# microsoft/DirectXTex

Measured on AMD Instinct MI355X. Metric: Mtexels/s BC7 encode (4096^2 RGBA8, TEX_COMPRESS_DEFAULT), higher is better.
Workload: dtype fp32 seed fit + i32 exact error sums (u8 texels in, 128-bit blocks out); 1 GPU; cfg2: 4096x4096 RGBA8 -> BC7_UNORM, TEX_COMPRESS_DEFAULT, one image per GPU, source and payload resident in HBM (dxtex_compress_device)

## Files before the change

directxtex_amd/csrc/bc7_encode.hip:

```cpp
#include "dxtex_kernels.h"
#include "bc67_tables.h"
#include "bc7_core.h"
#include "search_common.h"
#include <algorithm>
#include <cstdio>
#include <cstdlib>
#include <vector>

namespace dxtex
{
namespace
{
using namespace bc7;

struct Cand { uint32_t err; uint32_t ord; uint64_t lo, hi; };

enum : int { SLOT_M0 = 0, SLOT_M1, SLOT_M2, SLOT_M3, SLOT_M4A, SLOT_M4B, SLOT_M5, SLOT_M6, SLOT_M7, NUM_SLOTS };
enum : int { LIST_BYTES = 64 };

enum : int { PHASE_ALL = 0, PHASE_EARLY = 1, PHASE_LATE = 2 };

struct Bc7Args
{
    SegTable seg;
    uint32_t nblocks;
    uint32_t flags;
    uint8_t* lists;
    Cand* cands;
    uint32_t* px;
    struct TaskRec* recs;
    uint2* order;
    uint32_t* tinfo;
    uint32_t* counters;
    uint32_t* zeroOrd;
    uint2* seeds1;
    uint2* seeds3;
    uint2* seeds;
    int* bestErr;
    int prune;
    int alias;
    uint32_t* aliased;
    const uint32_t* flagged;
    uint32_t early6Min;
    uint32_t earlyAlphaMin;
    int early6Pct;
    int phase;
    const uint32_t* gate;
    uint32_t gateMin;
    uint32_t perturbWaveMax;
    uint32_t exhWaveMax;
};

constexpr uint32_t kWaveTaskMax = 262144;
constexpr uint32_t kWaveTaskMax45 = 24576;
constexpr uint32_t kPerturbWaveMax = 32768;

__device__ __forceinline__ void load_block_texel(const SrcView& src, uint32_t nbw, uint32_t nb, uint32_t t, float* f4, uint32_t& ldr)
{
    const uint32_t by = nb / nbw, bx = nb - by * nbw;
    const uint32_t x0 = bx * 4, y0 = by * 4;
    const uint32_t pw = min(4u, src.width - x0), ph = min(4u, src.height - y0);
    const uint32_t sx = x0 + replicate_src(t & 3, pw), sy = y0 + replicate_src(t >> 2, ph);
    const Texel px = convert_texel(load_texel(src.pixels + uint64_t(sy) * src.rowPitch, sx, src.format), src.tcv, src.tsw);
    f4[0] = px.r; f4[1] = px.g; f4[2] = px.b; f4[3] = px.a;
    const float c[4] = { px.r, px.g, px.b, px.a };
    ldr = 0;
#pragma unroll
    for (int i = 0; i < 4; ++i)
    {
        float v = c[i] * 255.0f + 0.01f;
        v = (v < 255.0f) ? v : 255.0f;
        v = (0.0f < v) ? v : 0.0f;
        ldr |= (uint32_t(v) & 0xFFu) << (8 * i);
    }
}

#if !defined(DXTEX_ROUGH_WGS)
#define DXTEX_ROUGH_WGS 8
#endif
__global__ void __launch_bounds__(256, DXTEX_ROUGH_WGS) bc7_rough_kernel(Bc7Args a)
{
    __shared__ float sF[4][64];
    __shared__ uint32_t sL[4][16];
    __shared__ uint2 sSeed[4][128];
    __shared__ int2 sErr[4][128];
    __shared__ uint32_t sOpaque[4];
    const int wave = threadIdx.x >> 6, lane = threadIdx.x & 63;
    const uint32_t nb = blockIdx.x * 4 + wave;
    const bool inRange = nb < a.nblocks;

    if (inRange && lane < 16)
    {
        uint32_t ldr;
        const BcSeg& sg = seg_of(a.seg, nb);
        load_block_texel(sg.src, sg.nbw, sg.nb0 + (nb - sg.l0), lane, &sF[wave][lane * 4], ldr);
        sL[wave][lane] = ldr;
        a.px[uint64_t(nb) * 16 + lane] = ldr;
        if (lane == 0) { a.zeroOrd[nb] = 0xFFFFFFFFu; a.bestErr[nb] = 0x7FFFFFFF; }
    }
    {
        const bool one = !inRange || lane >= 16 || sF[wave][(lane & 15) * 4 + 3] == 1.0f;
        const unsigned long long all = __ballot(one);
        if (lane == 0) sOpaque[wave] = (all == ~0ull) ? 1u : 0u;
    }
    __syncthreads();

    {
        const uint32_t blk = uint32_t(lane) >> 4, ent = uint32_t(lane) & 15u;
        const uint32_t nbk = blockIdx.x * 4 + blk;
        const float* fpxk = sF[blk];
        const uint32_t* pixk = sL[blk];
        const bool opaque = sOpaque[blk] != 0u;
#pragma unroll 1
        for (int k = 0; k < 2; ++k)
        {
            const uint32_t group = k ? uint32_t(7 - wave) : uint32_t(wave);
            const uint32_t code = kFit2Order[group * 16 + ent];
            if (nbk < a.nblocks)
            {
                const uint32_t m1 = kPart2Mask[code >> 1];
                const uint32_t m = (code & 1u) ? m1 : ((~m1) & 0xFFFFu);
                Region rg; region_init(rg, pixk, m);
                uint32_t A, B;
                if (rg.np == 1) { A = pixk[rg.pos(0)]; B = A; }
                else if (rg.np == 2) { A = pixk[rg.pos(0)]; B = pixk[rg.pos(1)]; }
                else if (opaque) seed_endpoints<true, false, true>(fpxk, m, A, B);
                else seed_endpoints<true>(fpxk, m, A, B);
                sSeed[blk][code] = make_uint2(A, B);
#if defined(DXTEX_ROUGH_SPLIT_ERR)
                sErr[blk][code] = make_int2(rough_error<3, 0>(rg, A, B), rough_error<2, 0>(rg, A, B));
#else
                int e3, e2;
                rough_error_3_2(rg, A, B, e3, e2);
                sErr[blk][code] = make_int2(e3, e2);
#endif
            }
        }
    }
    __syncthreads();
    if (!inRange) return;
    const float* fpx = sF[wave];
    const uint32_t* pix = sL[wave];

    const bool alphaLane = (lane < 16) && ((pix[lane & 15] >> 24) != 0xFFu);
    const bool hasAlpha = __ballot(alphaLane) != 0ull;

    uint8_t* lst = a.lists + uint64_t(nb) * LIST_BYTES;

    {
        const uint32_t shape = lane;
        const int2 er0 = sErr[wave][shape * 2], er1 = sErr[wave][shape * 2 + 1];
        const int e3 = er0.x + er1.x, e2 = er0.y + er1.y;
        int ea = e3, eb = e2;
        uint32_t sa = shape, sb = shape;
        for (int i = 0; i < 16; ++i)
        {
            selection_pass(ea, sa, lane, i);
            selection_pass(eb, sb, lane, i);
        }
        if (lane < 16) { lst[lane] = uint8_t(sa); lst[16 + lane] = uint8_t(sb); }
        {
            wave_lds_sync();
            uint32_t ranked2 = uint32_t(__shfl(int(sb), lane & 15));
            asm volatile("" : "+v"(ranked2));
            const uint32_t mine = (lane < 16) ? sa : ranked2;
            if (lane < 32)
            {
                const uint2 s0 = sSeed[wave][mine * 2], s1 = sSeed[wave][mine * 2 + 1];
                reinterpret_cast<uint4*>(a.seeds + uint64_t(nb) * 64)[lane] = make_uint4(s0.x, s0.y, s1.x, s1.y);
            }
        }
        if (lane == 0)
        {
            lst[32] = hasAlpha ? 1 : 0;
            *reinterpret_cast<int*>(lst + 56) = ea;
        }
    }

    if (a.flags & BCF_USE_3SUBSETS)
    {
        const uint32_t shape = lane;
        const uint32_t bits = kPart3Bits[shape];
        int e3 = 0, e2 = 0;
#pragma unroll 1
        for (uint32_t r = 0; r < 3; ++r)
        {
            uint32_t m = 0;
            for (int i = 0; i < 16; ++i) if (((bits >> (2 * i)) & 3u) == r) m |= 1u << i;
            Region rg; region_init(rg, pix, m);
            uint32_t A, B;
            if (rg.np == 1) { A = pix[rg.pos(0)]; B = A; }
            else if (rg.np == 2) { A = pix[rg.pos(0)]; B = pix[rg.pos(1)]; }
            else seed_endpoints<true>(fpx, m, A, B);
            a.seeds3[uint64_t(nb) * 192 + shape * 3 + r] = make_uint2(A, B);
            e3 += rough_error<3, 0>(rg, A, B);
            e2 += rough_error<2, 0>(rg, A, B);
        }
        int ea = (lane < 16) ? e3 : 0x7FFFFFFF, eb = e2;
        uint32_t sa = shape, sb = shape;
        for (int i = 0; i < 16; ++i)
        {
            if (i < 4) selection_pass(ea, sa, lane, i);
            selection_pass(eb, sb, lane, i);
        }
        if (lane < 4) lst[33 + lane] = uint8_t(sa);
        if (lane < 16) lst[40 + lane] = uint8_t(sb);
    }
}

struct TaskRec { uint32_t A, B; int err; int orgErr; };

template<int MODE, int IM> struct TaskMap
{
    typedef ModeInfo<MODE> MI;
    enum : int { NS = MI::NS,
                 G = (NS == 1) ? 1 : (NS == 2) ? 2 : 4,
                 RANKS = (NS == 1) ? ((MODE == 6) ? 1 : 4) : ((MODE == 0) ? 4 : 16),
                 TPB = RANKS * G,
                 LIST = (MODE == 1) ? 0 : (MODE == 0) ? 33 : (MODE == 2) ? 40 : 16,
                 SLOT = (MODE == 0) ? SLOT_M0 : (MODE == 1) ? SLOT_M1 : (MODE == 2) ? SLOT_M2 : (MODE == 3) ? SLOT_M3 :
                        (MODE == 4) ? (IM ? SLOT_M4B : SLOT_M4A) : (MODE == 5) ? SLOT_M5 : (MODE == 6) ? SLOT_M6 : SLOT_M7 };
};

template<int MODE, int IM>
__device__ __forceinline__ uint32_t candidate_sub(uint32_t rank)
{
    return (TaskMap<MODE, IM>::NS == 1) ? ((MODE == 4) ? (rank * 2 + IM) * 16u : rank * 16u) : rank;
}
template<int MODE, int IM>
__device__ __forceinline__ uint32_t candidate_ord(uint32_t rank) { return uint32_t(MODE) * 128u + candidate_sub<MODE, IM>(rank); }

template<int MODE>
__device__ __forceinline__ bool phase_owns(const Bc7Args& a, uint32_t nb)
{
    if (a.phase == PHASE_ALL || (MODE != 4 && MODE != 5 && MODE != 6)) return true;
    const uint8_t* lst = a.lists + uint64_t(nb) * LIST_BYTES;
    const bool early = (MODE == 6) ? (lst[37] != 0 && a.flagged[0] >= a.early6Min) : (lst[32] != 0 && a.flagged[1] >= a.earlyAlphaMin);
    return early == (a.phase == PHASE_EARLY);
}

__device__ __forceinline__ bool lst_has_alpha(const Bc7Args& a, uint32_t nb) { return a.lists[uint64_t(nb) * LIST_BYTES + 32] != 0; }

template<int MODE, int IM>
__device__ __forceinline__ bool task_geometry(const Bc7Args& a, uint32_t nb, uint32_t r, uint32_t& shape, uint32_t& mask, uint32_t& anchor, uint32_t& rot)
{
    typedef TaskMap<MODE, IM> TM;
    shape = 0; mask = 0xFFFFu; anchor = 0; rot = 0;
    if (nb >= a.nblocks) return false;
    if (!phase_owns<MODE>(a, nb)) return false;
    const uint32_t rank = r / TM::G, region = r % TM::G;
    if (a.zeroOrd[nb] < candidate_ord<MODE, IM>(rank)) return false;
    if (TM::NS == 1) { rot = (MODE == 6) ? 0u : r; return true; }
    if (region >= uint32_t(TM::NS)) return false;
    const uint8_t* lst = a.lists + uint64_t(nb) * LIST_BYTES;
    if (MODE == 7 && lst[32] == 0) return false;
    shape = lst[TM::LIST + rank];
    if (TM::NS == 2)
    {
        const uint32_t m1 = kPart2Mask[shape];
        mask = region ? m1 : ((~m1) & 0xFFFFu);
        anchor = region ? uint32_t(kAnchor2[shape]) : 0u;
    }
    else
    {
        const uint32_t bits = kPart3Bits[shape];
        mask = 0;
#pragma unroll
        for (int i = 0; i < 16; ++i) if (((bits >> (2 * i)) & 3u) == region) mask |= 1u << i;
        anchor = (region == 0) ? 0u : (region == 1) ? uint32_t(kAnchor3[shape] & 15) : uint32_t(kAnchor3[shape] >> 4);
    }
    return true;
}

template<int MODE, int IM, bool ASSIGN = true>
__device__ __forceinline__ void task_org(const float* fpx, const uint32_t* pix, uint32_t mask, uint32_t anchor, uint32_t rot,
                                         SubsetResult& res, int& np, bool wantRegion, Region& rgOut, Block16& b16Out, const uint2* seed = nullptr)
{
    typedef TaskMap<MODE, IM> TM;
    if (TM::NS == 1)
    {
        block16_init(b16Out, pix, rot);
        uint32_t A, B;
        if (seed) { const uint2 sd = seed[(MODE == 6) ? 1 : 0]; A = sd.x; B = sd.y; }
        else if (MODE == 6) seed_endpoints<true>(fpx, 0xFFFFu, A, B);
        else seed_endpoints<false>(fpx, 0xFFFFu, A, B);
        if (MODE != 6)
        {
            uint32_t mn = 255, mx = 0;
#pragma unroll
            for (int i = 0; i < 16; ++i) { const uint32_t al = b16Out.px[i] >> 24; mn = min(mn, al); mx = max(mx, al); }
            A = (A & 0x00FFFFFFu) | (mn << 24);
            B = (B & 0x00FFFFFFu) | (mx << 24);
        }
        if (ASSIGN) refine_pre_err<MODE, IM>(b16Out, A, B, 0u, res);
        else fix_pbits<MODE>(quantize_endpoint<MODE>(A), quantize_endpoint<MODE>(B), res.orgA, res.orgB);
        np = 16;
    }
    else
    {
        region_init(rgOut, pix, mask);
        uint32_t A, B;
        if (seed) { const uint2 sd = *seed; A = sd.x; B = sd.y; }
        else if (rgOut.np == 1) { A = pix[rgOut.pos(0)]; B = A; }
        else if (rgOut.np == 2) { A = pix[rgOut.pos(0)]; B = pix[rgOut.pos(1)]; }
        else seed_endpoints<true>(fpx, mask, A, B);
        if (ASSIGN) refine_pre_err<MODE, IM>(rgOut, A, B, anchor, res);
        else fix_pbits<MODE>(quantize_endpoint<MODE>(A), quantize_endpoint<MODE>(B), res.orgA, res.orgB);
        np = rgOut.np;
    }
}

template<int BPW>
__device__ __forceinline__ void stage_packed(const Bc7Args& a, uint32_t nbFirst, int lane, uint32_t* sL)
{
    for (int t = lane; t < BPW * 16; t += 64)
    {
        const uint32_t nb = nbFirst + (uint32_t(t) >> 4);
        sL[t] = (nb < a.nblocks) ? a.px[uint64_t(nb) * 16 + (t & 15)] : 0u;
    }
    wave_lds_sync();
}

#if !defined(DXTEX_PP45_WGS)
#define DXTEX_PP45_WGS 1
#endif
template<int MODE, int IM>
__global__ void __launch_bounds__(256, (MODE == 4 || MODE == 5) ? DXTEX_PP45_WGS : 1) bc7_pre_kernel(Bc7Args a)
{
    typedef TaskMap<MODE, IM> TM;
    constexpr int BPW = (TM::TPB >= 64) ? 1 : 64 / TM::TPB;
    __shared__ uint32_t sL[4][BPW * 16];
// ... 758 lines not shown
__global__ void __launch_bounds__(64) bc7_exhaustive_wave_kernel(Bc7Args a)
{
    typedef LoopCfg<MODE, IM, CHSET> C;
    typedef TaskMap<MODE, IM> TM;
    static_assert(TM::NS == 1, "whole-block tasks only");
    __shared__ uint32_t sTex[16 * kSlotStride];
    const int lane = threadIdx.x;
    const uint32_t live = a.counters[34];
    if (live == 0 || live > a.exhWaveMax) return;
    for (uint32_t idx = blockIdx.x; idx < live; idx += gridDim.x)
    {
        const uint2 task = a.order[idx];
        const TaskRec rec = a.recs[task.x];
        SlotRegion rg;
        wave_lds_sync();
        search_pickup<MODE, IM>(a, task, &sTex[0], rg);
        wave_lds_sync();
        int other;
        const int base = loop_base<MODE, IM, CHSET>(rg, rec.A, rec.B, &other);
        if (loop_is_settled<CHSET>(rec.err, other)) continue;
        ExhState st; st.optA = rec.A; st.optB = rec.B; st.optErr = rec.err;
        st.o = st.i = st.oEnd = st.iEnd = st.lo = 0; st.iA = 0; st.o0 = 0; st.aleb = 0; st.omin = st.imin = 0; st.best = rec.err; st.bestCode = -1; st.ch = C::CH0;
        VarPal<C::N> vp;
#pragma unroll 1
        for (int ch = C::CH0; ch < C::CH1; ++ch)
        {
            st = exh_window<MODE, IM, CHSET>(st, ch);
            if (st.ch >= C::CH1) break;
            varpal_init<MODE, IM, CHSET>(vp, st.optA, st.optB, ch);
            const int oStart = st.o;
            uint64_t bestKey = ~0ull;
#pragma unroll 1
            for (int round = 0; round < 2; ++round)
            {
                const int c = lane + 64 * round;
                const int o = oStart + c / 11, i = st.lo + c % 11;
                const bool valid = c < 121 && o < st.oEnd && i < st.iEnd && i >= o;
                int e = 0x7FFFFFFF;
                if (valid)
                {
                    const int av = st.aleb ? o : i, bv = st.aleb ? i : o;
                    e = eval_var<MODE, IM, CHSET>(rg, vp, ch, unq1<C::PREC>(uint32_t(av)), unq1<C::PREC>(uint32_t(bv)), base);
                }
                const uint64_t key = valid ? ((uint64_t(uint32_t(e)) << 8) | uint32_t(c)) : ~0ull;
                bestKey = key < bestKey ? key : bestKey;
            }
#pragma unroll
            for (int d = 32; d > 0; d >>= 1)
            {
                const uint32_t lo = uint32_t(__shfl_xor(int(uint32_t(bestKey)), d)), hi = uint32_t(__shfl_xor(int(uint32_t(bestKey >> 32)), d));
                const uint64_t other = (uint64_t(hi) << 32) | lo;
                bestKey = other < bestKey ? other : bestKey;
            }
            if (bestKey != ~0ull)
            {
                const int e = int(uint32_t(bestKey >> 8)), c = int(bestKey & 0xFFu);
                if (e < st.best) { st.best = e; st.omin = oStart + c / 11; st.imin = st.lo + c % 11; }
            }
            st = exh_commit(st);
        }
        if (lane == 0)
        {
            TaskRec* r = a.recs + task.x;
            r->A = st.optA; r->B = st.optB; r->err = st.optErr;
        }
    }
}

template<int MODE, int IM>
__global__ void __launch_bounds__(256, (MODE == 4 || MODE == 5) ? DXTEX_PP45_WGS : 1) bc7_post_kernel(Bc7Args a)
{
    typedef TaskMap<MODE, IM> TM;
    constexpr int BPW = (TM::TPB >= 64) ? 1 : 64 / TM::TPB;
    __shared__ uint32_t sL[4][BPW * 16];
    const int wave = threadIdx.x >> 6, lane = threadIdx.x & 63;
    const uint32_t nbFirst = (blockIdx.x * 4 + wave) * BPW;
    if (nbFirst >= a.nblocks) return;
    if (a.gate && *a.gate < a.gateMin) return;
    const uint32_t blk = uint32_t(lane) / TM::TPB, r = uint32_t(lane) % TM::TPB;
    const uint32_t nb = nbFirst + blk;
    const uint32_t rank = r / TM::G, region = r % TM::G;
    uint32_t shape, mask, anchor, rot;
    const bool active = (blk < uint32_t(BPW)) && task_geometry<MODE, IM>(a, nb, r, shape, mask, anchor, rot);
    const bool mine = blk < uint32_t(BPW) && nb < a.nblocks && phase_owns<MODE>(a, nb);
    if (!__any(active))
    {
        if (mine && r == 0)
        {
            Cand c; c.err = 0xFFFFFFFFu; c.ord = 0xFFFFFFFFu; c.lo = 0; c.hi = 0;
            a.cands[uint64_t(nb) * NUM_SLOTS + TM::SLOT] = c;
        }
        return;
    }
    stage_packed<BPW>(a, nbFirst, lane, sL[wave]);

    SubsetResult res;
    res.orgErr = 0; res.optErr = 0; res.orgA = res.orgB = res.optA = res.optB = 0;
    res.orgIdx1 = res.orgIdx2 = res.optIdx1 = res.optIdx2 = 0;
    int np = 0; Region rg; Block16 b16;
    if (active)
    {
        task_org<MODE, IM, false>(nullptr, &sL[wave][blk * 16], mask, anchor, rot, res, np, true, rg, b16,
                                  (TM::NS == 2) ? a.seeds + uint64_t(nb) * 64 + (TM::LIST ? 32 : 0) + r
                                                : (TM::NS == 1) ? a.seeds1 + uint64_t(nb) * 2 : a.seeds3 + uint64_t(nb) * 192 + shape * 3 + (r % TM::G));
        TaskRec rec = a.recs[uint64_t(nb) * TM::TPB + r];
        if constexpr (TM::NS >= 2)
        {
            const uint32_t leader = (a.tinfo[uint64_t(nb) * TM::TPB + r] >> 18) & 63u;
            if (leader)
            {
                const TaskRec lead = a.recs[uint64_t(nb) * TM::TPB + (leader - 1u)];
                rec.A = lead.A; rec.B = lead.B;
            }
        }
        res.orgErr = rec.orgErr;
        if (TM::NS == 1) refine_post<MODE, IM>(b16, rec.A, rec.B, 0u, res);
        else refine_post<MODE, IM>(rg, rec.A, rec.B, anchor, res);
    }
    int orgTot = res.orgErr, optTot = res.optErr;
#pragma unroll
    for (int d = 1; d < TM::G; d <<= 1) { orgTot += __shfl_xor(orgTot, d); optTot += __shfl_xor(optTot, d); }
    const bool useOpt = optTot < orgTot;
    const int err = useOpt ? optTot : orgTot;
    const uint32_t sub = candidate_sub<MODE, IM>(rank);
    const uint32_t key = active ? ((uint32_t(err) << 7) | sub) : 0xFFFFFFFFu;
    uint32_t best = key;
#pragma unroll
    for (int d = 1; d < TM::TPB && d < 64; d <<= 1) best = min(best, uint32_t(__shfl_xor(int(best), d)));
    const bool needOrg = active && key == best && !useOpt;
    if (__any(needOrg))
    {
        if (needOrg)
        {
            if (TM::NS == 1) (void)assign_indices<MODE, IM>(b16, res.orgA, res.orgB, 0u, res.orgIdx1, res.orgIdx2);
            else (void)assign_indices<MODE, IM>(rg, res.orgA, res.orgB, anchor, res.orgIdx1, res.orgIdx2);
        }
    }
    const uint32_t myA = useOpt ? res.optA : res.orgA, myB = useOpt ? res.optB : res.orgB;
    const uint64_t myIdx1 = useOpt ? res.optIdx1 : res.orgIdx1, myIdx2 = useOpt ? res.optIdx2 : res.orgIdx2;
    uint32_t epA[3] = { myA, 0, 0 }, epB[3] = { myB, 0, 0 };
    uint64_t idx1 = myIdx1;
#pragma unroll
    for (int s = 1; s < TM::NS; ++s)
    {
        epA[s] = uint32_t(__shfl_down(int(myA), s));
        epB[s] = uint32_t(__shfl_down(int(myB), s));
        const uint64_t oi = uint64_t(uint32_t(__shfl_down(int(uint32_t(myIdx1)), s))) |
                            (uint64_t(uint32_t(__shfl_down(int(uint32_t(myIdx1 >> 32)), s))) << 32);
        idx1 |= oi;
    }

    if (blk < uint32_t(BPW) && nb < a.nblocks && region == 0)
    {
        if (active && key == best)
        {
            uint32_t anchors[3] = { 0, 0, 0 };
            if (TM::NS == 2) anchors[1] = kAnchor2[shape];
            if (TM::NS == 3) { anchors[1] = kAnchor3[shape] & 15; anchors[2] = kAnchor3[shape] >> 4; }
            Cand c;
            c.err = uint32_t(err);
            c.ord = uint32_t(MODE) * 128u + sub;
            emit_block<MODE>(shape, rot, IM, epA, epB, idx1, myIdx2, anchors, c.lo, c.hi);
            a.cands[uint64_t(nb) * NUM_SLOTS + TM::SLOT] = c;
            if (err == 0) atomicMin(&a.zeroOrd[nb], c.ord);
            atomicMin(&a.bestErr[nb], err);
        }
        else if (!active && rank == 0 && mine)
        {
            Cand c; c.err = 0xFFFFFFFFu; c.ord = 0xFFFFFFFFu; c.lo = 0; c.hi = 0;
            a.cands[uint64_t(nb) * NUM_SLOTS + TM::SLOT] = c;
        }
    }
}

template<bool RGBA>
__global__ void __launch_bounds__(256) bc7_block_seeds_kernel(Bc7Args a)
{
    const uint32_t nb = blockIdx.x * 256u + threadIdx.x;
    if (nb >= a.nblocks) return;
    const BcSeg& sg = seg_of(a.seg, nb);
    float f[64];
#pragma unroll
    for (int t = 0; t < 16; ++t) { uint32_t ldr; load_block_texel(sg.src, sg.nbw, sg.nb0 + (nb - sg.l0), uint32_t(t), &f[t * 4], ldr); }
    uint32_t A, B;
    seed_endpoints<RGBA, true>(f, 0xFFFFu, A, B);
    a.seeds1[uint64_t(nb) * 2 + (RGBA ? 1 : 0)] = make_uint2(A, B);
}

__global__ void __launch_bounds__(256) bc7_flag_count_kernel(Bc7Args a, uint32_t* out)
{
    uint32_t n = 0, m = 0;
    for (uint32_t nb = blockIdx.x * 256u + threadIdx.x; nb < a.nblocks; nb += gridDim.x * 256u)
    {
        uint8_t* lst = a.lists + uint64_t(nb) * LIST_BYTES;
        const bool hasAlpha = lst[32] != 0;
        bool first = hasAlpha;
        if (!first)
        {
            const uint4* px4 = reinterpret_cast<const uint4*>(a.px + uint64_t(nb) * 16);
            const uint4 q0 = px4[0], q1 = px4[1], q2 = px4[2], q3 = px4[3];
            const uint32_t px[16] = { q0.x, q0.y, q0.z, q0.w, q1.x, q1.y, q1.z, q1.w, q2.x, q2.y, q2.z, q2.w, q3.x, q3.y, q3.z, q3.w };
            const int ea = *reinterpret_cast<const int*>(lst + 56);
            first = int64_t(subset_lower_bound(px, 0xFFFFu, 0u, 4)) * 100 <= int64_t(ea) * a.early6Pct;
        }
        lst[37] = first ? 1 : 0;
        n += first ? 1u : 0u;
        m += hasAlpha ? 1u : 0u;
    }
#pragma unroll
    for (int o = 32; o > 0; o >>= 1) { n += __shfl_xor(n, o); m += __shfl_xor(m, o); }
    if ((threadIdx.x & 63u) == 0 && n) atomicAdd(out, n);
    if ((threadIdx.x & 63u) == 0 && m) atomicAdd(out + 1, m);
}

__global__ void __launch_bounds__(256) bc7_texels_kernel(Bc7Args a)
{
    const uint32_t i = blockIdx.x * 256u + threadIdx.x;
    if (i >= a.nblocks * 16u) return;
    float f4[4]; uint32_t ldr;
    const BcSeg& sg = seg_of(a.seg, i >> 4);
    load_block_texel(sg.src, sg.nbw, sg.nb0 + ((i >> 4) - sg.l0), i & 15u, f4, ldr);
    a.px[i] = ldr;
    if ((i & 15u) == 0) { a.zeroOrd[i >> 4] = 0xFFFFFFFFu; a.bestErr[i >> 4] = 0x7FFFFFFF; }
}

__global__ void __launch_bounds__(256) bc7_pick_kernel(Bc7Args a, uint32_t slotMask)
{
    const uint32_t nb = blockIdx.x * 256u + threadIdx.x;
    if (nb >= a.nblocks) return;
    const Cand* c = a.cands + uint64_t(nb) * NUM_SLOTS;
    uint64_t bestKey = ~0ull;
    uint64_t lo = 0, hi = 0;
#pragma unroll
    for (int s = 0; s < NUM_SLOTS; ++s)
    {
        if (!((slotMask >> s) & 1u)) continue;
        if (s == SLOT_M7 && a.flagged[1] == 0) continue;
        const Cand v = c[s];
        if (v.err == 0xFFFFFFFFu) continue;
        const uint64_t key = (uint64_t(v.err) << 32) | v.ord;
        if (key < bestKey) { bestKey = key; lo = v.lo; hi = v.hi; }
    }
    const BcSeg& sg = seg_of(a.seg, nb);
    const uint32_t gb = sg.nb0 + (nb - sg.l0);
    const uint32_t by = gb / sg.nbw, bx = gb - by * sg.nbw;
    uint64_t* out = reinterpret_cast<uint64_t*>(sg.dst + uint64_t(by) * sg.dstRowPitch) + 2 * uint64_t(bx);
    out[0] = lo; out[1] = hi;
}
}

namespace
{
const uint64_t kMaxBlocksPerPass = dev_env("DXTEX_MAX_BLOCKS_PER_PASS") ? std::max<uint64_t>(1, strtoull(dev_env("DXTEX_MAX_BLOCKS_PER_PASS"), nullptr, 10)) : (1u << 22);
constexpr int kMaxTasksPerBlock = 64;
const uint64_t kSmallPassBlocks = dev_env("DXTEX_BC7_SMALL_BLOCKS") ? strtoull(dev_env("DXTEX_BC7_SMALL_BLOCKS"), nullptr, 10) : 262144;
struct ScratchLayout
{
    size_t lists, cands, px, recs, order, tinfo, counters, zeroOrd, bestErr, seeds, seeds1, seeds3, flagcnt, auxRecs, auxOrder, auxTinfo, auxCounters, total;
    size_t auxTpb, auxSlices;
    explicit ScratchLayout(uint64_t nb, bool threeSubsets)
    {
        auto up = [](size_t v) { return (v + 255) & ~size_t(255); };
        const size_t tpb = threeSubsets ? kMaxTasksPerBlock : 32;
        const bool small = nb <= kSmallPassBlocks;
        auxTpb = small ? tpb : 4; auxSlices = small ? size_t(kSideStreams) : 2;
        size_t o = 0;
        lists = o; o = up(o + nb * LIST_BYTES);
        cands = o; o = up(o + nb * NUM_SLOTS * sizeof(Cand));
        px = o; o = up(o + nb * 64);
        recs = o; o = up(o + nb * tpb * sizeof(TaskRec));
        order = o; o = up(o + nb * tpb * sizeof(uint2));
        tinfo = o; o = up(o + nb * tpb * sizeof(uint32_t));
        counters = o; o = up(o + 64 * sizeof(uint32_t));
        zeroOrd = o; o = up(o + nb * sizeof(uint32_t));
        bestErr = o; o = up(o + nb * sizeof(int));
        seeds = o; o = up(o + nb * 64 * sizeof(uint2));
        seeds1 = o; o = up(o + nb * 2 * sizeof(uint2));
        seeds3 = o; o = up(o + (threeSubsets ? nb * 192 * sizeof(uint2) : 0));
        flagcnt = o; o = up(o + 256);
        auxRecs = o; o = up(o + auxSlices * nb * auxTpb * sizeof(TaskRec));
        auxOrder = o; o = up(o + auxSlices * nb * auxTpb * sizeof(uint2));
        auxTinfo = o; o = up(o + auxSlices * nb * auxTpb * sizeof(uint32_t));
        auxCounters = o; o = up(o + size_t(kSideStreams) * 64 * sizeof(uint32_t));
        total = o;
    }
};

template<int MODE, int IM>
void launch_mode(const Bc7Args& a0, hipStream_t stream, KernelMarks* marks, const char* const (&names)[7])
{
    typedef TaskMap<MODE, IM> TM;
    constexpr int BPW = (TM::TPB >= 64) ? 1 : 64 / TM::TPB;
    const uint32_t nb = a0.nblocks;
    const uint32_t ntasks = nb * uint32_t(TM::TPB);
    const uint32_t gridPP = (nb + 4 * BPW - 1) / (4 * BPW);
    constexpr bool kWhole = TM::NS == 1;
    constexpr uint32_t kExhMax = (MODE == 6) ? kWaveTaskMax : kWaveTaskMax45;
    static const bool noGroup = dev_env("DXTEX_BC7_NO_GROUP") != nullptr;
    const bool maybeShortP = kWhole && !noGroup && (MODE == 6 || ntasks <= 4u * kPerturbWaveMax);
    const bool maybeShortE = kWhole && !noGroup && (MODE == 6 || ntasks <= 4u * kExhMax);
    const uint32_t wavesP = std::min<uint32_t>(kSearchWaves, (ntasks + 1) / 2), wavesE = std::min<uint32_t>(kSearchWaves, ntasks);
    Bc7Args a = a0;
    a.gate = nullptr; a.gateMin = 0;
    if (a0.flagged && !(a0.flags & BCF_BC7_QUICK))
    {
        if (MODE == 7) { a.gate = a0.flagged + 1; a.gateMin = 1; }
        else if (a0.phase == PHASE_EARLY && (MODE == 4 || MODE == 5)) { a.gate = a0.flagged + 1; a.gateMin = std::max<uint32_t>(1u, a0.earlyAlphaMin); }
        else if (a0.phase == PHASE_EARLY && MODE == 6) { a.gate = a0.flagged; a.gateMin = std::max<uint32_t>(1u, a0.early6Min); }
    }
    a.perturbWaveMax = maybeShortP ? kPerturbWaveMax : 0u;
    a.exhWaveMax = maybeShortE ? kExhMax : 0u;
    if (marks) marks->mark(names[0]);
    hipLaunchKernelGGL((bc7_pre_kernel<MODE, IM>), dim3(gridPP), dim3(256), 0, stream, a);
    if (marks) marks->mark(names[1]);
    (void)hipMemsetAsync(a.counters, 0, 64 * sizeof(uint32_t), stream);
    const uint32_t binGroups = std::min<uint32_t>(kBinGroups, (ntasks + 255) / 256);
    hipLaunchKernelGGL(bc7_bin_count_kernel, dim3(binGroups), dim3(256), 0, stream, a.tinfo, ntasks, a.counters, a.gate, a.gateMin);
    hipLaunchKernelGGL(bc7_bin_scan_kernel, dim3(1), dim3(1), 0, stream, a.counters);
    hipLaunchKernelGGL(bc7_bin_scatter_kernel, dim3(binGroups), dim3(256), 0, stream, a.tinfo, ntasks, a.counters, a.order, a.gate, a.gateMin);
    if (marks) marks->mark(names[2]);
    const uint32_t waves = std::min<uint32_t>(kSearchWaves, (ntasks + 63) / 64);
    static const int tailBelow = dev_env("DXTEX_BC7_TAIL_BELOW") ? atoi(dev_env("DXTEX_BC7_TAIL_BELOW")) : 48;
    static const bool perturbPlain = dev_env("DXTEX_BC7_PERTURB_PLAIN") != nullptr;
    static const int rangeTests = dev_env("DXTEX_BC7_NO_PEEL") ? 3 : ((dev_env("DXTEX_BC7_RANGE_TESTS") ? atoi(dev_env("DXTEX_BC7_RANGE_TESTS")) & 0xFF : DXTEX_RANGE_TESTS) |
                                                                       ((dev_env("DXTEX_BC7_PEEL_LAYERS") ? atoi(dev_env("DXTEX_BC7_PEEL_LAYERS")) : 1) << 8));
    if constexpr (PaletteBits<MODE, IM>::AB == 0)
    {
        if constexpr (MODE == 1 || MODE == 6)
        {
            if (perturbPlain) hipLaunchKernelGGL((bc7_perturb_kernel<MODE, IM, CH_ALL>), dim3(waves), dim3(64), 0, stream, a, 0);
            else hipLaunchKernelGGL((bc7_perturb_filter_kernel<MODE, IM, CH_ALL>), dim3(waves), dim3(64), 0, stream, a, 0);
        }
        else
            hipLaunchKernelGGL((bc7_perturb_kernel<MODE, IM, CH_ALL>), dim3(waves), dim3(64), 0, stream, a, 0);
        if constexpr (kWhole) { if (maybeShortP) hipLaunchKernelGGL((bc7_perturb_wave_kernel<MODE, IM, CH_ALL>), dim3(wavesP), dim3(64), 0, stream, a); }
        if (marks) marks->mark(names[4]);
        if constexpr (kWhole) { if (maybeShortE) hipLaunchKernelGGL((bc7_exhaustive_wave_kernel<MODE, IM, CH_ALL>), dim3(wavesE), dim3(64), 0, stream, a); }
        hipLaunchKernelGGL((bc7_exhaustive_kernel<MODE, IM, CH_ALL>), dim3(waves), dim3(64), 0, stream, a, 1, tailBelow, rangeTests);
    }
    else
    {
        if constexpr (MODE == 4 && IM == 1 && DXTEX_PF_M4 != 0)
        {
            if (perturbPlain) hipLaunchKernelGGL((bc7_perturb_kernel<MODE, IM, CH_COLOR>), dim3(waves), dim3(64), 0, stream, a, 0);
            else hipLaunchKernelGGL((bc7_perturb_filter_kernel<MODE, IM, CH_COLOR>), dim3(waves), dim3(64), 0, stream, a, 0);
        }
        else
            hipLaunchKernelGGL((bc7_perturb_kernel<MODE, IM, CH_COLOR>), dim3(waves), dim3(64), 0, stream, a, 0);
        if (maybeShortP) hipLaunchKernelGGL((bc7_perturb_wave_kernel<MODE, IM, CH_COLOR>), dim3(wavesP), dim3(64), 0, stream, a);
        if (marks) marks->mark(names[3]);
        hipLaunchKernelGGL((bc7_perturb_kernel<MODE, IM, CH_ALPHA>), dim3(waves), dim3(64), 0, stream, a, 1);
        if (maybeShortP) hipLaunchKernelGGL((bc7_perturb_wave_kernel<MODE, IM, CH_ALPHA>), dim3(wavesP), dim3(64), 0, stream, a);
        if (marks) marks->mark(names[4]);
        if (maybeShortE) hipLaunchKernelGGL((bc7_exhaustive_wave_kernel<MODE, IM, CH_COLOR>), dim3(wavesE), dim3(64), 0, stream, a);
        hipLaunchKernelGGL((bc7_exhaustive_kernel<MODE, IM, CH_COLOR>), dim3(waves), dim3(64), 0, stream, a, 2, tailBelow, rangeTests);
        if (marks) marks->mark(names[5]);
        if (maybeShortE) hipLaunchKernelGGL((bc7_exhaustive_wave_kernel<MODE, IM, CH_ALPHA>), dim3(wavesE), dim3(64), 0, stream, a);
        hipLaunchKernelGGL((bc7_exhaustive_kernel<MODE, IM, CH_ALPHA>), dim3(waves), dim3(64), 0, stream, a, 3, tailBelow, rangeTests);
    }
    if (marks) marks->mark(names[6]);
    hipLaunchKernelGGL((bc7_post_kernel<MODE, IM>), dim3(gridPP), dim3(256), 0, stream, a);
#if defined(DXTEX_DEV)
    static const bool stats = dev_env("DXTEX_BC7_STATS") != nullptr;
    if (stats)
    {
        uint32_t c[40] = {};
// ... 64 lines not shown
            const unsigned long long* e = w + idx[idx.size() / 2] * WT_FIELDS;
            std::fprintf(stderr, "    median wavefront %d: start %.0f drained %.0f end %.0f %% of span, rounds %llu, busy lanes / round %.1f, tasks %llu\n", idx[idx.size() / 2],
                         100.0 * double(e[0] - t0) / dur, 100.0 * double(e[1] - t0) / dur, 100.0 * double(e[2] - t0) / dur, e[3], e[3] ? double(e[4]) / e[3] : 0.0, e[5]);
        }
    }
    std::fill(h.begin(), h.end(), 0ull); std::fill(hist.begin(), hist.end(), 0u);
    (void)hipMemcpyToSymbol(HIP_SYMBOL(g_wt), h.data(), h.size() * 8);
    (void)hipMemcpyToSymbol(HIP_SYMBOL(g_wtHist), hist.data(), hist.size() * 4);
}
}
#endif

size_t bc7_scratch_bytes(uint64_t nblocks, uint32_t flags, size_t nimages)
{
    const bool three = (flags & BCF_USE_3SUBSETS) != 0;
    size_t need = ScratchLayout(nblocks < kMaxBlocksPerPass ? nblocks : kMaxBlocksPerPass, three).total;
    if (nblocks > kSmallPassBlocks) need = std::max(need, ScratchLayout(kSmallPassBlocks, three).total);
    return need + seg_table_bytes(nblocks, kMaxBlocksPerPass, nimages);
}

hipError_t launch_bc7_encode(const SrcView& src, uint8_t* dst, uint64_t dstRowPitch, uint32_t flags,
                             void* scratch, hipStream_t stream, KernelMarks* marks, const SideStreams* side)
{
    BcImage one; one.src = src; one.dst = dst; one.dstRowPitch = dstRowPitch;
    return launch_bc7_encode_many(&one, 1, flags, scratch, stream, marks, side);
}

hipError_t launch_bc7_encode_many(const BcImage* images, size_t count, uint32_t flags, void* scratch, hipStream_t stream, KernelMarks* marks,
                                  const SideStreams* side)
{
#define DXTEX_MARK(NAME) do { if (marks) marks->mark(NAME); } while (0)
#define DXTEX_MODE(MODE, IM, TAG) do { static const char* const n_[7] = { "bc7_pre_" TAG, "bc7_bin_" TAG, "bc7_perturb_" TAG, "bc7_perturb_alpha_" TAG, \
                                           "bc7_exhaustive_" TAG, "bc7_exhaustive_alpha_" TAG, "bc7_post_" TAG }; \
                                       launch_mode<MODE, IM>(a, stream, marks, n_); } while (0)
    std::vector<BcSeg> segs;
    std::vector<BcPass> passes;
    uint64_t perPass = 0;
    if (!build_passes(images, count, kMaxBlocksPerPass, segs, passes, &perPass)) return hipSuccess;
    const bool three = (flags & BCF_USE_3SUBSETS) != 0;
    const ScratchLayout L(perPass, three);
    uint8_t* base = static_cast<uint8_t*>(scratch);
    BcSeg* dSegs = reinterpret_cast<BcSeg*>(base + L.total);
    const hipError_t ce = upload_segments(dSegs, segs, passes, stream);
    if (ce != hipSuccess) return ce;
    const bool quick = (flags & BCF_BC7_QUICK) != 0;

    for (const BcPass& pass : passes)
    {
        Bc7Args a;
        set_pass(a.seg, dSegs, segs, pass);
        a.nblocks = pass.nblocks;
        a.flags = flags;
        a.perturbWaveMax = 0; a.exhWaveMax = 0;
        a.gate = nullptr; a.gateMin = 0;
        a.lists = base + L.lists;
        a.cands = reinterpret_cast<Cand*>(base + L.cands);
        a.px = reinterpret_cast<uint32_t*>(base + L.px);
        a.recs = reinterpret_cast<TaskRec*>(base + L.recs);
        a.order = reinterpret_cast<uint2*>(base + L.order);
        a.tinfo = reinterpret_cast<uint32_t*>(base + L.tinfo);
        a.counters = reinterpret_cast<uint32_t*>(base + L.counters);
        a.zeroOrd = reinterpret_cast<uint32_t*>(base + L.zeroOrd);
        a.bestErr = reinterpret_cast<int*>(base + L.bestErr);
        a.seeds = reinterpret_cast<uint2*>(base + L.seeds);
        a.seeds1 = reinterpret_cast<uint2*>(base + L.seeds1);
        a.seeds3 = reinterpret_cast<uint2*>(base + L.seeds3);
        static const bool noPrune = dev_env("DXTEX_BC7_NO_PRUNE") != nullptr;
        a.prune = noPrune ? 0 : 1;
        static const bool noAlias = dev_env("DXTEX_BC7_NO_ALIAS") != nullptr;
        a.alias = noAlias ? 0 : 1;
        static const int early6 = dev_env("DXTEX_BC7_EARLY6_PCT") ? atoi(dev_env("DXTEX_BC7_EARLY6_PCT")) : 100;
        a.early6Pct = early6;
        uint32_t slotMask = 0;

        uint32_t* flagCount = reinterpret_cast<uint32_t*>(base + L.flagcnt);
        a.flagged = flagCount;
        a.aliased = flagCount + 48;
        static const int early6MinPct = dev_env("DXTEX_BC7_EARLY6_MIN_PCT") ? atoi(dev_env("DXTEX_BC7_EARLY6_MIN_PCT")) : -1;
        static const int earlyAlphaMinPct = dev_env("DXTEX_BC7_EARLYA_MIN_PCT") ? atoi(dev_env("DXTEX_BC7_EARLYA_MIN_PCT")) : 25;
        const bool smallPlanRuns = side && !marks && !quick && dev_env("DXTEX_BC7_SERIAL") == nullptr && dev_env("DXTEX_BC7_NO_SMALL_PLAN") == nullptr &&
                                   L.auxTpb >= 32 && perPass <= kSmallPassBlocks && dev_env("DXTEX_BC7_ORDER") == nullptr;
        a.early6Min = uint32_t(uint64_t(a.nblocks) * uint32_t(early6MinPct >= 0 ? early6MinPct : (smallPlanRuns ? 25 : 50)) / 100u);
        a.earlyAlphaMin = uint32_t(uint64_t(a.nblocks) * uint32_t(earlyAlphaMinPct) / 100u);
        if (!quick)
        {
            DXTEX_MARK("bc7_rough");
            hipLaunchKernelGGL(bc7_rough_kernel, dim3((a.nblocks + 3) / 4), dim3(256), 0, stream, a);
            (void)hipMemsetAsync(flagCount, 0, 256, stream);
            hipLaunchKernelGGL(bc7_flag_count_kernel, dim3((a.nblocks + 255) / 256), dim3(256), 0, stream, a, flagCount);
        }
        else
        {
            DXTEX_MARK("bc7_texels");
            hipLaunchKernelGGL(bc7_texels_kernel, dim3((a.nblocks * 16 + 255) / 256), dim3(256), 0, stream, a);
        }
        DXTEX_MARK("bc7_block_seeds");
        if (!quick) hipLaunchKernelGGL(bc7_block_seeds_kernel<false>, dim3((a.nblocks + 255) / 256), dim3(256), 0, stream, a);
        hipLaunchKernelGGL(bc7_block_seeds_kernel<true>, dim3((a.nblocks + 255) / 256), dim3(256), 0, stream, a);
        static const std::vector<int> order = []
        {
            std::vector<int> o;
            const char* e = dev_env("DXTEX_BC7_ORDER");
            const char* p = e ? e : "16,7,14,18,15,0,1,2,3,24,28,25,26";
            while (*p)
            {
                if (*p >= '0' && *p <= '9') { o.push_back(int(strtol(p, const_cast<char**>(&p), 10))); }
                else ++p;
            }
            return o;
        }();
        a.phase = PHASE_ALL;
        if (quick) { DXTEX_MODE(6, 0, "mode6"); slotMask |= 1u << SLOT_M6; }
        auto run_step = [&](int step, Bc7Args a, hipStream_t stream, KernelMarks* marks)
        {
            a.phase = (step >= 20) ? PHASE_LATE : (step >= 10) ? PHASE_EARLY : PHASE_ALL;
            switch (step)
            {
            case 0: DXTEX_MODE(0, 0, "mode0"); slotMask |= 1u << SLOT_M0; break;
            case 1: DXTEX_MODE(1, 0, "mode1"); slotMask |= 1u << SLOT_M1; break;
            case 2: DXTEX_MODE(2, 0, "mode2"); slotMask |= 1u << SLOT_M2; break;
            case 3: DXTEX_MODE(3, 0, "mode3"); slotMask |= 1u << SLOT_M3; break;
            case 4: DXTEX_MODE(4, 0, "mode4_im0"); slotMask |= 1u << SLOT_M4A; break;
            case 14: DXTEX_MODE(4, 0, "mode4_im0_early"); slotMask |= 1u << SLOT_M4A; break;
            case 24: DXTEX_MODE(4, 0, "mode4_im0_late"); slotMask |= 1u << SLOT_M4A; break;
            case 8: DXTEX_MODE(4, 1, "mode4_im1"); slotMask |= 1u << SLOT_M4B; break;
            case 18: DXTEX_MODE(4, 1, "mode4_im1_early"); slotMask |= 1u << SLOT_M4B; break;
            case 28: DXTEX_MODE(4, 1, "mode4_im1_late"); slotMask |= 1u << SLOT_M4B; break;
            case 5: DXTEX_MODE(5, 0, "mode5"); slotMask |= 1u << SLOT_M5; break;
            case 15: DXTEX_MODE(5, 0, "mode5_early"); slotMask |= 1u << SLOT_M5; break;
            case 25: DXTEX_MODE(5, 0, "mode5_late"); slotMask |= 1u << SLOT_M5; break;
            case 6: DXTEX_MODE(6, 0, "mode6"); slotMask |= 1u << SLOT_M6; break;
            case 16: DXTEX_MODE(6, 0, "mode6_early"); slotMask |= 1u << SLOT_M6; break;
            case 26: DXTEX_MODE(6, 0, "mode6_late"); slotMask |= 1u << SLOT_M6; break;
            case 7: DXTEX_MODE(7, 0, "mode7"); slotMask |= 1u << SLOT_M7; break;
            default: break;
            }
        };
        auto family45 = [](int step) { const int m = step % 10; return m == 4 || m == 8 || m == 5; };
        static const bool serial45 = dev_env("DXTEX_BC7_SERIAL") != nullptr;
        const SideStreams* fork = (marks || serial45 || quick) ? nullptr : side;
        auto side_args = [&](const Bc7Args& a0, size_t k)
        {
            Bc7Args b = a0;
            b.recs = reinterpret_cast<TaskRec*>(base + L.auxRecs) + k * size_t(a0.nblocks) * L.auxTpb;
            b.order = reinterpret_cast<uint2*>(base + L.auxOrder) + k * size_t(a0.nblocks) * L.auxTpb;
            b.tinfo = reinterpret_cast<uint32_t*>(base + L.auxTinfo) + k * size_t(a0.nblocks) * L.auxTpb;
            b.counters = reinterpret_cast<uint32_t*>(base + L.auxCounters) + k * 64;
            return b;
        };
        static const std::vector<std::vector<std::vector<int>>> smallPlan = []
        {
            const char* e = dev_env("DXTEX_BC7_SMALL_PLAN");
            const char* p = e ? e : "1,26/3,2/16,14,15,18,7,0|24/28/25";
            std::vector<std::vector<std::vector<int>>> stages(1, std::vector<std::vector<int>>(1));
            while (*p)
            {
                if (*p >= '0' && *p <= '9') stages.back().back().push_back(int(strtol(p, const_cast<char**>(&p), 10)));
                else
                {
                    if (*p == '|') stages.emplace_back(1);
                    else if (*p == '/' && stages.back().size() < size_t(kSideStreams) + 1) stages.back().emplace_back();
                    ++p;
                }
            }
            return stages;
        }();
        static const bool noSmall = dev_env("DXTEX_BC7_NO_SMALL_PLAN") != nullptr;
        if (fork && !noSmall && smallPlanRuns)
        {
            for (const std::vector<std::vector<int>>& stage : smallPlan)
            {
// ... 52 lines not shown
```

Before: 144.8 Mtexels/s.

## Deduplicate identical BC7 blocks with a hash table and reuse leader results

```diff
diff --git a/directxtex_amd/csrc/bc7_encode.hip b/directxtex_amd/csrc/bc7_encode.hip
--- a/directxtex_amd/csrc/bc7_encode.hip
+++ b/directxtex_amd/csrc/bc7_encode.hip
@@ -1,6 +1,7 @@
 #include "dxtex_kernels.h"
 #include "bc67_tables.h"
 #include "bc7_core.h"
+#include "dxtex_bc7_dedupe.h"
 #include "search_common.h"
 #include <algorithm>
 #include <cstdio>
@@ -49,7 +50,15 @@
     uint32_t gateMin;
     uint32_t perturbWaveMax;
     uint32_t exhWaveMax;
+    uint32_t* dupOf;
+    bc7dd::Slot* ddTable;
+    uint32_t ddSlots;
+    uint32_t ddHashBits;
+    int dedupe;
+    uint32_t* ddCount;
 };
+
+__device__ __forceinline__ bool is_duplicate(const Bc7Args& a, uint32_t nb) { return a.dupOf[nb] != nb; }
 
 constexpr uint32_t kWaveTaskMax = 262144;
 constexpr uint32_t kWaveTaskMax45 = 24576;
@@ -75,6 +84,76 @@
     }
 }
 
+__global__ void __launch_bounds__(256) bc7_dedupe_insert_kernel(Bc7Args a)
+{
+    const uint32_t nb = blockIdx.x * 256u + threadIdx.x;
+    const int lane = threadIdx.x & 63;
+    const bool valid = nb < a.nblocks;
+    uint64_t h = 0;
+    if (valid)
+    {
+        const BcSeg& sg = seg_of(a.seg, nb);
+#pragma unroll 4
+        for (uint32_t t = 0; t < 16; ++t)
+        {
+            float f4[4]; uint32_t ldr;
+            load_block_texel(sg.src, sg.nbw, sg.nb0 + (nb - sg.l0), t, f4, ldr);
+#pragma unroll
+            for (int c = 0; c < 4; ++c) h = bc7dd::hash_word(h, __float_as_uint(f4[c]));
+        }
+    }
+    const unsigned long long key = bc7dd::hash_finish(h, a.ddHashBits);
+    int first = lane;
+    for (int j = 0; j < 63; ++j)
+    {
+        const unsigned long long kj = (unsigned long long)(uint32_t(__shfl(int(uint32_t(key)), j))) |
+                                      ((unsigned long long)(uint32_t(__shfl(int(uint32_t(key >> 32)), j))) << 32);
+        if (first == lane && j < lane && kj == key) first = j;
+    }
+    uint32_t slot = bc7dd::kNoSlot;
+    if (valid && first == lane)
+    {
+        bc7dd::Slot* table = a.ddTable;
+        slot = bc7dd::insert(key, nb, a.ddSlots,
+                             [table](uint32_t s, unsigned long long k) { return atomicCAS(&table[s].key, bc7dd::kEmptyKey, k); },
+                             [table](uint32_t s, uint32_t b) { atomicMin(&table[s].leader, b); });
+    }
+    slot = uint32_t(__shfl(int(slot), first));
+    if (valid) a.dupOf[nb] = slot;
+}
+
+__global__ void __launch_bounds__(256) bc7_dedupe_resolve_kernel(Bc7Args a)
+{
+    const uint32_t nb = blockIdx.x * 256u + threadIdx.x;
+    const bool valid = nb < a.nblocks;
+    uint32_t leader = nb;
+    if (valid && a.dedupe)
+    {
+        const uint32_t cand = bc7dd::candidate_leader(a.ddTable, a.dupOf[nb], nb);
+        if (cand != nb)
+        {
+            const BcSeg& sg = seg_of(a.seg, nb);
+            const BcSeg& sl = seg_of(a.seg, cand);
+            uint32_t diff = 0;
+#pragma unroll 1
+            for (uint32_t t = 0; t < 16 && diff == 0; ++t)
+            {
+                float f[4], g[4]; uint32_t ldr;
+                load_block_texel(sg.src, sg.nbw, sg.nb0 + (nb - sg.l0), t, f, ldr);
+                load_block_texel(sl.src, sl.nbw, sl.nb0 + (cand - sl.l0), t, g, ldr);
+#pragma unroll
+                for (int c = 0; c < 4; ++c) diff |= __float_as_uint(f[c]) ^ __float_as_uint(g[c]);
+            }
+            if (diff == 0) leader = cand;
+        }
+    }
+    if (valid) a.dupOf[nb] = leader;
+#if defined(DXTEX_DEV)
+    const unsigned long long dups = __ballot(valid && leader != nb);
+    if (dups && (threadIdx.x & 63u) == 0) atomicAdd(a.ddCount, uint32_t(__popcll(dups)));
+#endif
+}
+
 #if !defined(DXTEX_ROUGH_WGS)
 #define DXTEX_ROUGH_WGS 8
 #endif
@@ -88,8 +167,9 @@
     const int wave = threadIdx.x >> 6, lane = threadIdx.x & 63;
     const uint32_t nb = blockIdx.x * 4 + wave;
     const bool inRange = nb < a.nblocks;
-
-    if (inRange && lane < 16)
+    const bool dup = inRange && is_duplicate(a, nb);
+
+    if (inRange && !dup && lane < 16)
     {
         uint32_t ldr;
         const BcSeg& sg = seg_of(a.seg, nb);
@@ -99,7 +179,7 @@
         if (lane == 0) { a.zeroOrd[nb] = 0xFFFFFFFFu; a.bestErr[nb] = 0x7FFFFFFF; }
     }
     {
-        const bool one = !inRange || lane >= 16 || sF[wave][(lane & 15) * 4 + 3] == 1.0f;
+        const bool one = !inRange || dup || lane >= 16 || sF[wave][(lane & 15) * 4 + 3] == 1.0f;
         const unsigned long long all = __ballot(one);
         if (lane == 0) sOpaque[wave] = (all == ~0ull) ? 1u : 0u;
     }
@@ -111,12 +191,13 @@
         const float* fpxk = sF[blk];
         const uint32_t* pixk = sL[blk];
         const bool opaque = sOpaque[blk] != 0u;
+        const bool fitted = nbk < a.nblocks && !is_duplicate(a, nbk);
 #pragma unroll 1
         for (int k = 0; k < 2; ++k)
         {
             const uint32_t group = k ? uint32_t(7 - wave) : uint32_t(wave);
             const uint32_t code = kFit2Order[group * 16 + ent];
-            if (nbk < a.nblocks)
+            if (fitted)
             {
                 const uint32_t m1 = kPart2Mask[code >> 1];
                 const uint32_t m = (code & 1u) ? m1 : ((~m1) & 0xFFFFu);
@@ -138,7 +219,7 @@
         }
     }
     __syncthreads();
-    if (!inRange) return;
+    if (!inRange || dup) return;
     const float* fpx = sF[wave];
     const uint32_t* pix = sL[wave];
 
@@ -246,7 +327,7 @@
 {
     typedef TaskMap<MODE, IM> TM;
     shape = 0; mask = 0xFFFFu; anchor = 0; rot = 0;
-    if (nb >= a.nblocks) return false;
+    if (nb >= a.nblocks || is_duplicate(a, nb)) return false;
     if (!phase_owns<MODE>(a, nb)) return false;
     const uint32_t rank = r / TM::G, region = r % TM::G;
     if (a.zeroOrd[nb] < candidate_ord<MODE, IM>(rank)) return false;
@@ -1171,7 +1252,7 @@
     const uint32_t rank = r / TM::G, region = r % TM::G;
     uint32_t shape, mask, anchor, rot;
     const bool active = (blk < uint32_t(BPW)) && task_geometry<MODE, IM>(a, nb, r, shape, mask, anchor, rot);
-    const bool mine = blk < uint32_t(BPW) && nb < a.nblocks && phase_owns<MODE>(a, nb);
+    const bool mine = blk < uint32_t(BPW) && nb < a.nblocks && !is_duplicate(a, nb) && phase_owns<MODE>(a, nb);
     if (!__any(active))
     {
         if (mine && r == 0)
@@ -1266,7 +1347,7 @@
 __global__ void __launch_bounds__(256) bc7_block_seeds_kernel(Bc7Args a)
 {
     const uint32_t nb = blockIdx.x * 256u + threadIdx.x;
-    if (nb >= a.nblocks) return;
+    if (nb >= a.nblocks || is_duplicate(a, nb)) return;
     const BcSeg& sg = seg_of(a.seg, nb);
     float f[64];
 #pragma unroll
@@ -1281,6 +1362,7 @@
     uint32_t n = 0, m = 0;
     for (uint32_t nb = blockIdx.x * 256u + threadIdx.x; nb < a.nblocks; nb += gridDim.x * 256u)
     {
+        if (is_duplicate(a, nb)) continue;
         uint8_t* lst = a.lists + uint64_t(nb) * LIST_BYTES;
         const bool hasAlpha = lst[32] != 0;
         bool first = hasAlpha;
@@ -1305,7 +1387,7 @@
 __global__ void __launch_bounds__(256) bc7_texels_kernel(Bc7Args a)
 {
     const uint32_t i = blockIdx.x * 256u + threadIdx.x;
-    if (i >= a.nblocks * 16u) return;
+    if (i >= a.nblocks * 16u || is_duplicate(a, i >> 4)) return;
     float f4[4]; uint32_t ldr;
     const BcSeg& sg = seg_of(a.seg, i >> 4);
     load_block_texel(sg.src, sg.nbw, sg.nb0 + ((i >> 4) - sg.l0), i & 15u, f4, ldr);
@@ -1317,7 +1399,7 @@
 {
     const uint32_t nb = blockIdx.x * 256u + threadIdx.x;
     if (nb >= a.nblocks) return;
-    const Cand* c = a.cands + uint64_t(nb) * NUM_SLOTS;
+    const Cand* c = a.cands + uint64_t(a.dupOf[nb]) * NUM_SLOTS;
     uint64_t bestKey = ~0ull;
     uint64_t lo = 0, hi = 0;
 #pragma unroll
@@ -1345,7 +1427,7 @@
 const uint64_t kSmallPassBlocks = dev_env("DXTEX_BC7_SMALL_BLOCKS") ? strtoull(dev_env("DXTEX_BC7_SMALL_BLOCKS"), nullptr, 10) : 262144;
 struct ScratchLayout
 {
-    size_t lists, cands, px, recs, order, tinfo, counters, zeroOrd, bestErr, seeds, seeds1, seeds3, flagcnt, auxRecs, auxOrder, auxTinfo, auxCounters, total;
+    size_t lists, cands, px, recs, order, tinfo, counters, zeroOrd, bestErr, seeds, seeds1, seeds3, flagcnt, auxRecs, auxOrder, auxTinfo, auxCounters, dupOf, ddTable, total;
     size_t auxTpb, auxSlices;
     explicit ScratchLayout(uint64_t nb, bool threeSubsets)
     {
@@ -1371,6 +1453,8 @@
         auxOrder = o; o = up(o + auxSlices * nb * auxTpb * sizeof(uint2));
         auxTinfo = o; o = up(o + auxSlices * nb * auxTpb * sizeof(uint32_t));
         auxCounters = o; o = up(o + size_t(kSideStreams) * 64 * sizeof(uint32_t));
+        dupOf = o; o = up(o + nb * sizeof(uint32_t));
+        ddTable = o; o = up(o + nb * bc7dd::kSlotsPerBlock * sizeof(bc7dd::Slot));
         total = o;
     }
 };
@@ -1601,11 +1685,36 @@
                                    L.auxTpb >= 32 && perPass <= kSmallPassBlocks && dev_env("DXTEX_BC7_ORDER") == nullptr;
         a.early6Min = uint32_t(uint64_t(a.nblocks) * uint32_t(early6MinPct >= 0 ? early6MinPct : (smallPlanRuns ? 25 : 50)) / 100u);
         a.earlyAlphaMin = uint32_t(uint64_t(a.nblocks) * uint32_t(earlyAlphaMinPct) / 100u);
+        static const bool noDedupe = dev_env("DXTEX_BC7_NO_DEDUPE") != nullptr;
+        static const int hashBits = dev_env("DXTEX_BC7_DEDUPE_HASH_BITS") ? atoi(dev_env("DXTEX_BC7_DEDUPE_HASH_BITS")) : 64;
+        a.dupOf = reinterpret_cast<uint32_t*>(base + L.dupOf);
+        a.ddTable = reinterpret_cast<bc7dd::Slot*>(base + L.ddTable);
+        a.ddSlots = a.nblocks * bc7dd::kSlotsPerBlock;
+        a.ddHashBits = uint32_t(std::min(64, std::max(0, hashBits)));
+        a.dedupe = noDedupe ? 0 : 1;
+        a.ddCount = flagCount + 60;
+        DXTEX_MARK("bc7_dedupe");
+        (void)hipMemsetAsync(flagCount, 0, 256, stream);
+        if (a.dedupe)
+        {
+            (void)hipMemsetAsync(a.ddTable, 0xFF, size_t(a.ddSlots) * sizeof(bc7dd::Slot), stream);
+            hipLaunchKernelGGL(bc7_dedupe_insert_kernel, dim3((a.nblocks + 255) / 256), dim3(256), 0, stream, a);
+        }
+        hipLaunchKernelGGL(bc7_dedupe_resolve_kernel, dim3((a.nblocks + 255) / 256), dim3(256), 0, stream, a);
+#if defined(DXTEX_DEV)
+        static const bool ddStats = dev_env("DXTEX_BC7_STATS") != nullptr;
+        if (ddStats)
+        {
+            uint32_t dups = 0;
+            (void)hipStreamSynchronize(stream);
+            (void)hipMemcpy(&dups, a.ddCount, sizeof(dups), hipMemcpyDeviceToHost);
+            std::fprintf(stderr, "bc7 stats dedupe: %u of %u blocks are duplicates\n", dups, a.nblocks);
+        }
+#endif
         if (!quick)
         {
             DXTEX_MARK("bc7_rough");
             hipLaunchKernelGGL(bc7_rough_kernel, dim3((a.nblocks + 3) / 4), dim3(256), 0, stream, a);
-            (void)hipMemsetAsync(flagCount, 0, 256, stream);
             hipLaunchKernelGGL(bc7_flag_count_kernel, dim3((a.nblocks + 255) / 256), dim3(256), 0, stream, a, flagCount);
         }
         else
diff --git a/directxtex_amd/csrc/dxtex_bc7_dedupe.h b/directxtex_amd/csrc/dxtex_bc7_dedupe.h
--- /dev/null
+++ b/directxtex_amd/csrc/dxtex_bc7_dedupe.h
@@ -0,0 +1,83 @@
+#pragma once
+#include <cstdint>
+
+#if defined(__HIP__) || defined(__CUDACC__)
+#define DXTEX_DD_HD __host__ __device__
+#else
+#define DXTEX_DD_HD
+#endif
+
+namespace dxtex
+{
+namespace bc7dd
+{
+constexpr uint32_t kKeyWords = 64;
+constexpr unsigned long long kEmptyKey = ~0ull;
+constexpr uint32_t kNoSlot = 0xFFFFFFFFu;
+constexpr uint32_t kProbeBound = 32;
+constexpr uint32_t kSlotsPerBlock = 2;
+
+struct Slot { unsigned long long key; uint32_t leader; uint32_t pad; };
+
+DXTEX_DD_HD inline uint64_t mix64(uint64_t x)
+{
+    x ^= x >> 30; x *= 0xBF58476D1CE4E5B9ull;
+    x ^= x >> 27; x *= 0x94D049BB133111EBull;
+    return x ^ (x >> 31);
+}
+
+DXTEX_DD_HD inline uint64_t hash_word(uint64_t h, uint32_t w)
+{
+    h = (h ^ w) * 0x9E3779B97F4A7C15ull;
+    return h ^ (h >> 29);
+}
+
+DXTEX_DD_HD inline unsigned long long hash_finish(uint64_t h, uint32_t bits)
+{
+    h = mix64(h);
+    if (bits < 64u) h &= (1ull << bits) - 1ull;
+    return (h == kEmptyKey) ? 0ull : h;
+}
+
+DXTEX_DD_HD inline unsigned long long hash_key(const uint32_t* words, uint32_t bits)
+{
+    uint64_t h = 0;
+    for (uint32_t i = 0; i < kKeyWords; ++i) h = hash_word(h, words[i]);
+    return hash_finish(h, bits);
+}
+
+DXTEX_DD_HD inline uint32_t slot_start(unsigned long long h, uint32_t slots)
+{
+    return uint32_t(((mix64(h ^ 0xD6E8FEB86659FD93ull) >> 32) * uint64_t(slots)) >> 32);
+}
+DXTEX_DD_HD inline uint32_t slot_at(uint32_t start, uint32_t i, uint32_t slots) { return (start + i) % slots; }
+
+template<class Cas, class Amin>
+DXTEX_DD_HD inline uint32_t insert(unsigned long long h, uint32_t nb, uint32_t slots, Cas cas, Amin amin)
+{
+    const uint32_t start = slot_start(h, slots);
+    const uint32_t bound = (slots < kProbeBound) ? slots : kProbeBound;
+    for (uint32_t i = 0; i < bound; ++i)
+    {
+        const uint32_t s = slot_at(start, i, slots);
+        const unsigned long long prev = cas(s, h);
+        if (prev == kEmptyKey || prev == h) { amin(s, nb); return s; }
+    }
+    return kNoSlot;
+}
+
+DXTEX_DD_HD inline uint32_t candidate_leader(const Slot* table, uint32_t slot, uint32_t nb)
+{
+    if (slot == kNoSlot) return nb;
+    const uint32_t l = table[slot].leader;
+    return (l < nb) ? l : nb;
+}
+
+DXTEX_DD_HD inline bool keys_equal(const uint32_t* x, const uint32_t* y)
+{
+    uint32_t diff = 0;
+    for (uint32_t i = 0; i < kKeyWords; ++i) diff |= x[i] ^ y[i];
+    return diff == 0;
+}
+}
+}
```

Result: faster. 153.0 Mtexels/s, median of 6 (+5.7%).
